# WZN1ng/Cooperative-Search

Hardware: AMD Instinct MI355X
Metric: env-steps/sec (higher is better)
Workload: dtype f64

## Files before the change

### cooperative-search_amd/csrc/rollout_oct.h

```cpp

#ifndef CS_OCT_PREFILTER
#define CS_OCT_PREFILTER 0
#endif
constexpr int OCT_WAVES = 3;
constexpr int OG = 8;
constexpr int OCT_ENVS = 64 / OG;
constexpr int OCT_BLOCK = 256;
constexpr int OCT_PAD = CS_MAX_AGENTS + 1;

struct __attribute__((aligned(16))) OctShared {
    double2 pos[OCT_ENVS][OCT_PAD];
    double2 tgt[OCT_ENVS][CS_MAX_TARGETS];
    float tile[OCT_ENVS * TILE_W];
    float reward[OCT_ENVS];
    int term[OCT_ENVS], win[OCT_ENVS];
    unsigned rowbuf[MT_N];
};

template <int LG>
struct OctLay;
template <>
struct OctLay<8> {
    static constexpr int ENVS = 8, TPL = 2;
    static constexpr unsigned SLICE = 0xffu;
// ... 96 lines not shown
};

struct OctKin {
    double cx, cy;
    double c1, s1;
    double xf, yf;
    bool hitf;
    bool hit;
};

__device__ __forceinline__ void div2_same_denominator(double nx, double ny, double den, double &qx, double &qy) {
    const double LO = 0x1p-100, HI = 0x1p100;
    const int e_lo = min(__builtin_amdgcn_frexp_exp(nx), __builtin_amdgcn_frexp_exp(ny));
    const bool plain = (den >= LO) & (den <= HI) & (fabs(nx) <= HI) & (fabs(ny) <= HI) & (e_lo >= -99);
    if (__builtin_expect(__ballot(!plain) == 0ull, 1)) {
        double r = __builtin_amdgcn_rcp(den);
        r = __builtin_fma(__builtin_fma(-den, r, 1.0), r, r);
        r = __builtin_fma(__builtin_fma(-den, r, 1.0), r, r);
        const double mx = nx * r, my = ny * r;
        qx = __builtin_fma(__builtin_fma(-den, mx, nx), r, mx);
        qy = __builtin_fma(__builtin_fma(-den, my, ny), r, my);
        return;
    }
    qx = nx / den;
    qy = ny / den;
}

template <int N, int I, bool SHARED_DIV, int LG = OG>
struct OctStage {
    static __device__ __forceinline__ void run(const DevParams &p, const double2 (&pre)[N], int t, bool act_lane,
                                               unsigned long long act_mask, OctKin &k) {
        if constexpr (I < N) {
            const double2 pi = pre[I];
            const double xi = pi.x, yi = pi.y;
            const double dx = k.cx - xi, dy = k.cy - yi;
            const double d2 = dx * dx + dy * dy;
            const bool c_lt = d2 < p.force_d2;
            const unsigned long long not_i = ~OctLay<LG>::lanes_t(I);
            if (__ballot(c_lt) & act_mask & not_i) {
                const bool c_nx = k.cx != xi, c_ny = k.cy != yi;
                const bool inr = act_lane & (t != I) & c_lt & (c_nx | c_ny);
                const double ex = -dx, ey = -dy;
                const double den = d2;
                double qx, qy;
                if constexpr (SHARED_DIV) {
                    div2_same_denominator(p.force_k * ex, p.force_k * ey, inr ? den : 1.0, qx, qy);
                } else {
                    qx = p.force_k * ex / den;
                    qy = p.force_k * ey / den;
                }
                const double tx = inr ? qx : 0.0;
                const double ty = inr ? qy : 0.0;
                double fx = 0.0, fy = 0.0;
                OctForceSum<N, I>::run(tx, ty, fx, fy);
                const double x = (k.cx + p.velocity * k.c1) + fx;
                const double y = (k.cy + p.velocity * k.s1) + fy;
                const bool h = (x < 0.0) | (x > p.L) | (y < 0.0) | (y > p.L);
                if (t == I) {
                    k.cx = h ? fmin(fmax(x, 0.0), p.L) : x;
                    k.cy = h ? fmin(fmax(y, 0.0), p.L) : y;
                    k.hit = h;
                }
            } else if (t == I) {
                k.cx = k.xf;
                k.cy = k.yf;
                k.hit = k.hitf;
            }
            OctStage<N, I + 1, SHARED_DIV, LG>::run(p, pre, t, act_lane, act_mask, k);
        }
    }
};

template <int N, bool SHARED_DIV = false, int LG = OG, int AP = OCT_PAD>
__device__ __forceinline__ unsigned oct_kinematics(const DevParams &p, const double *T, const double2 (*pos)[AP], int o, int t,
                                                   int sh8, bool stepping, int act, EnvO<N, LG> &e, int tl_step = -1) {
    static_assert(LG == OG, "one layout: the octet");
    const double PI = 3.141592653589793, TWO_PI = 2.0 * 3.141592653589793, THREE_PI = 3.0 * 3.141592653589793;
    const double DYAW = 3.141592653589793 / 18.0;
    const bool upd = (t < N) & stepping;
    double2 pre[N];
#pragma unroll
    for (int I = 0; I < N; I++) pre[I] = pos[o][I];
    double yaw = e.yaw;
    yaw = act == 1 ? yaw + DYAW : (act == 2 ? yaw + -DYAW : yaw);
    yaw = yaw > TWO_PI ? yaw - TWO_PI : (yaw < 0.0 ? yaw + TWO_PI : yaw);
    const double yw = yaw, yr = (yaw <= PI) ? PI - yaw : THREE_PI - yaw;
    double s1, c1, s2, c2;
    KIN_STAMP(3);
    if constexpr (N <= 4) {
        const double yr_up = dpp_f64<0x114>(yr);
        double sm, cm;
        trig_heading(T, t >= 4 ? yr_up : yw, sm, cm);
        s1 = sm;
        c1 = cm;
        s2 = dpp_f64<0x104>(sm);
        c2 = dpp_f64<0x104>(cm);
    } else {
        trig_heading_pair(T, yw, yr, s1, c1, s2, c2);
    }
    KIN_STAMP(4);
    const double xt = (e.x + p.velocity * c1) + 0.0, yt = (e.y + p.velocity * s1) + 0.0;
    const bool hitf = (xt < 0.0) | (xt > p.L) | (yt < 0.0) | (yt > p.L);
    OctKin k{e.x, e.y, c1, s1, hitf ? fmin(fmax(xt, 0.0), p.L) : xt, hitf ? fmin(fmax(yt, 0.0), p.L) : yt, hitf, false};
    constexpr bool FASTPATH = N <= 3;
    bool any_pair = !FASTPATH;
#pragma unroll
    for (int I = 0; I < (FASTPATH ? N : 0); I++) {
        const double2 pi = pre[I];
        const double qx = t < I ? k.xf : e.x, qy = t < I ? k.yf : e.y;
        const double dx = qx - pi.x, dy = qy - pi.y;
        any_pair = any_pair | ((t != I) & (dx * dx + dy * dy < p.force_d2) & ((qx != pi.x) | (qy != pi.y)));
    }
    const unsigned long long upd_mask = __ballot(upd);
    if (FASTPATH ? __ballot(any_pair & upd) != 0ull : upd_mask != 0ull) {
        OctStage<N, 0, SHARED_DIV, LG>::run(p, pre, t, upd, upd_mask, k);
    } else {
        k.cx = k.xf;
        k.cy = k.yf;
        k.hit = k.hitf;
    }
    KIN_STAMP(5);
    e.x = upd ? k.cx : e.x;
    e.y = upd ? k.cy : e.y;
    e.yaw = upd ? (k.hit ? yr : yw) : e.yaw;
    e.cs = upd ? (k.hit ? c2 : c1) : e.cs;
    e.sn = upd ? (k.hit ? s2 : s1) : e.sn;
    return oct_slice<LG>(__ballot(k.hit & upd), sh8);
}

__device__ __forceinline__ void tape_canon(unsigned (&t)[TAPE_DW], int &tcur) {
#pragma unroll
    for (int k = 0; k < TAPE_DW; k++) t[k] = __builtin_amdgcn_alignbit(k + 1 < TAPE_DW ? t[k + 1] : 0u, t[k], (unsigned)tcur);
    tcur = 0;
}
template <int N, int LG, int AP, bool LAZY, bool PRE = false>
__device__ __forceinline__ int oct_detect_impl(const DevParams &p, const double2 (*pos)[AP], int o, int t, int sh8, bool stepping,
                                               EnvO<N, LG> &e, unsigned (&tape)[TAPE_DW], int &tcur, const float *nrow = nullptr,
                                               int nstride = 0) {
    constexpr int MAXDW = (N * CS_MAX_TARGETS) / 32 < 1 ? 1 : (N * CS_MAX_TARGETS) / 32;
    constexpr int TPL = OctLay<LG>::TPL;
    static_assert(!PRE || TPL == 2, "the packed pre-filter holds a lane's two targets in one register pair");
    bool has[TPL], inr[N][TPL];
    unsigned below[TPL];
    int rank[N][TPL];
    int base = 0;
#pragma unroll
    for (int k = 0; k < TPL; k++) {
        has[k] = stepping & (t + LG * k < p.n_targets);
        below[k] = (1u << (t + LG * k)) - 1u;
    }
    auto exact = [&]() __attribute__((always_inline)) {
#pragma unroll
        for (int i = 0; i < N; i++) {
            const double2 a = pos[o][i];
#pragma unroll
            for (int k = 0; k < TPL; k++) {
                const double dx = e.tx[k] - a.x, dy = e.ty[k] - a.y;
                inr[i][k] = has[k] & (dx * dx + dy * dy <= p.view_r2);
            }
        }
    };
    if constexpr (PRE) {
        typedef float pk2 __attribute__((ext_vector_type(2)));
        const pk2 tnx = {e.tnx[0], e.tnx[1]}, tny = {e.tny[0], e.tny[1]};
        const float thr = p.thr32;
        float margin = 3.0e38f;
#pragma unroll
        for (int i = 0; i < N; i++) {
            const float ax = nrow[nstride * i], ay = nrow[nstride * i + 1];
            const pk2 dx = tnx - pk2{ax, ax}, dy = tny - pk2{ay, ay};
            const pk2 d2 = __builtin_elementwise_fma(dx, dx, dy * dy);
            const pk2 u = d2 - pk2{thr, thr};
            inr[i][0] = has[0] & (u[0] < 0.0f);
            inr[i][1] = has[1] & (u[1] < 0.0f);
            margin = __builtin_fminf(margin, __builtin_fminf(__builtin_fabsf(u[0]), __builtin_fabsf(u[1])));
        }
#ifndef CS_PREFILTER_EPS_SCALE
#define CS_PREFILTER_EPS_SCALE 1.0f
#endif
        if (__builtin_expect(__ballot(margin <= p.eps32 * CS_PREFILTER_EPS_SCALE) != 0ull, 0)) exact();
    } else {
        exact();
    }
#pragma unroll
    for (int i = 0; i < N; i++) {
        unsigned gm = 0u;
#pragma unroll
        for (int k = 0; k < TPL; k++) gm |= oct_slice<LG>(__ballot(inr[i][k]), sh8) << (LG * k);
#pragma unroll
        for (int k = 0; k < TPL; k++) rank[i][k] = base + __popc(gm & below[k]);
        base += __popc(gm);
    }
    unsigned w4[4];
#pragma unroll
    for (int k = 0; k < 4; k++) w4[k] = LAZY ? __builtin_amdgcn_alignbit(tape[k + 1], tape[k], (unsigned)tcur) : tape[k];
    const unsigned long long t64a = (unsigned long long)w4[0] | ((unsigned long long)w4[1] << 32);
    const unsigned long long t64b = (unsigned long long)w4[2] | ((unsigned long long)w4[3] << 32);
    auto slot = [&](int r) __attribute__((always_inline)) {
        if (N * CS_MAX_TARGETS <= 64) return (bool)((t64a >> r) & 1ull);
        return (bool)(((r >= 64 ? t64b : t64a) >> (r & 63)) & 1ull);
    };
    bool hit[TPL];
#pragma unroll
    for (int k = 0; k < TPL; k++) hit[k] = false;
    if (N * CS_MAX_TARGETS <= 64 || __builtin_expect(__ballot(base > 64) == 0ull, 1)) {
#pragma unroll
        for (int i = 0; i < N; i++)
#pragma unroll
            for (int k = 0; k < TPL; k++) hit[k] = hit[k] | (inr[i][k] & (bool)((t64a >> rank[i][k]) & 1ull));
    } else {
#pragma unroll
        for (int i = 0; i < N; i++)
#pragma unroll
            for (int k = 0; k < TPL; k++) hit[k] = hit[k] | (inr[i][k] & slot(rank[i][k]));
    }
    e.mt_pos = wrap624(e.mt_pos + 2 * base);
    e.words += (unsigned long long)(2 * base);
    e.ahead -= 2 * base;
    if constexpr (LAZY) {
        tcur += base;
#pragma unroll
        for (int r = 0; r <= MAXDW; r++) {
            const bool out = tcur >= 32;
            if (__ballot(out) == 0ull) break;
#pragma unroll
            for (int k = 0; k < TAPE_DW; k++) tape[k] = out ? (k + 1 < TAPE_DW ? tape[k + 1] : 0u) : tape[k];
            tcur -= out ? 32 : 0;
        }
    } else {
        tape_shift<MAXDW>(tape, base);
    }
    unsigned newly = 0u;
#pragma unroll
    for (int k = 0; k < TPL; k++) {
        const bool nw = hit[k] & !((e.found >> (t + LG * k)) & 1u);
        newly |= oct_slice<LG>(__ballot(nw), sh8) << (LG * k);
    }
    int r = 0;
    if (stepping) {
        const int cnt = __popc(newly);
        r = -1 + 10 * cnt;
        e.found |= newly;
        e.newly = newly;
        e.target_find += cnt;
        if (cnt > 0 && e.target_find == p.n_targets && !(e.flags & FLAG_WIN)) {
            r += 100;
            e.flags |= FLAG_WIN;
        }
        r -= __popc(((unsigned)e.flags >> 8) & 0xffu);
        e.curr_reward = r;
        e.flags |= FLAG_DIRTY;
    }
    return r;
}
template <int N, int LG = OG, int AP = OCT_PAD>
__device__ __forceinline__ int oct_detect(const DevParams &p, const double2 (*pos)[AP], int o, int t, int sh8, bool stepping,
                                          EnvO<N, LG> &e, unsigned (&tape)[TAPE_DW]) {
    int zero = 0;
    return oct_detect_impl<N, LG, AP, false>(p, pos, o, t, sh8, stepping, e, tape, zero);
}

template <int N, bool DRAIN = true, int LG = OG>
__device__ __forceinline__ void oct_wave_advance(const DevParams &p, int wave_b0, int nvalid, int lane, int min_ahead,
                                                 unsigned *rowbuf, EnvO<N, LG> &e, unsigned (&tape)[TAPE_DW], bool &tape_ok) {
    const int o = OctLay<LG>::valid(lane) ? OctLay<LG>::env(lane) : -1;
#pragma unroll 1
    for (int g = 0; g < OctLay<LG>::ENVS; g++) {
        const int pos = __shfl(e.mt_pos, OctLay<LG>::first_of(g)), a = __shfl(e.ahead, OctLay<LG>::first_of(g));
        const int ok = __shfl(tape_ok ? 1 : 0, OctLay<LG>::first_of(g));
        if (g >= nvalid || (ok && a >= min_ahead)) continue;
        unsigned *m = p.mt + (size_t)(wave_b0 + g) * MT_STRIDE;
        RowRegs rr;
        row_load(m, lane, rr);
        row_to_lds(rr, rowbuf, lane);
        row_twist_ahead(rowbuf, m, pos, a < 0 ? 0 : a, lane);
        unsigned long long bms[TAPE_DW / 2];
        row_hits_all(p, rowbuf, pos, lane, bms);
#pragma unroll
        for (int it = 0; it < TAPE_DW / 2; it++) {
            const unsigned long long bm = bms[it];
            if (o == g) {
                tape[2 * it] = (unsigned)(bm & 0xffffffffull);
                tape[2 * it + 1] = (unsigned)(bm >> 32);
            }
        }
        if (o == g) {
            e.ahead = MT_N;
            tape_ok = true;
        }
    }
    if (DRAIN) drain_vmem();
}


template <int N, int LG = OG>
__device__ __forceinline__ void oct_advance_finish(const DevParams &p, int wave_b0, int g, int lane, unsigned *rowbuf,
                                                   EnvO<N, LG> &e, unsigned (&tape)[TAPE_DW], bool &tape_ok) {
    const int o = OctLay<LG>::valid(lane) ? OctLay<LG>::env(lane) : -1;
    const int pos = __shfl(e.mt_pos, OctLay<LG>::first_of(g)), a = __shfl(e.ahead, OctLay<LG>::first_of(g));
    row_twist_ahead(rowbuf, p.mt + (size_t)(wave_b0 + g) * MT_STRIDE, pos, a < 0 ? 0 : a, lane);
    unsigned long long bms[TAPE_DW / 2];
    row_hits_all(p, rowbuf, pos, lane, bms);
#pragma unroll
    for (int it = 0; it < TAPE_DW / 2; it++) {
        const unsigned long long bm = bms[it];
        if (o == g) {
            tape[2 * it] = (unsigned)(bm & 0xffffffffull);
            tape[2 * it + 1] = (unsigned)(bm >> 32);
        }
    }
    if (o == g) {
        e.ahead = MT_N;
        tape_ok = true;
    }
}

template <int N, bool DRAIN, int LG = OG, class BeforeTile, class Pre>
__device__ __forceinline__ void oct_place_targets(const DevParams &cp, int wave_b0, int nvalid, int lane, bool live,
                                                  unsigned long long need, const double *rtab, double2 (*slots)[G], float *tile,
                                                  int W, unsigned *rowbuf, EnvO<N, LG> &e, unsigned (&tape)[TAPE_DW], bool &tape_ok,
                                                  BeforeTile before_tile, Pre pre) {
    using Lay = OctLay<LG>;
    const CS_AS4 DevParams *q = cold_params4();
    const int t16 = lane & (G - 1), gshift16 = lane & ~(G - 1), grp = lane >> 4, sh8 = Lay::first(lane), t = Lay::t(lane);
    const int n_targets = q->n_targets, target_mode = q->target_mode;
    const unsigned deter_mask = q->deter_mask;
    const double mid = q->mid, inv_half = q->inv_half, L = q->L;
    const CS_AS1 unsigned *mt = (const CS_AS1 unsigned *)q->mt;
    CS_AS1 double *tgt = (CS_AS1 double *)q->tgt;
    const unsigned tmask = n_targets >= 32 ? ~0u : ((1u << n_targets) - 1u);
    const unsigned fmask = target_mode == 0 ? ~deter_mask & tmask : 0u;
    const int need_total = __popc(fmask);
    const bool jit = (fmask >> t16) & 1u;
    const int my_rank = __popc(fmask & ((1u << t16) - 1u));
    unsigned long long pend = need;
    int taken_env = 0;
    bool first = true;
    while (pend) {
        const bool pending = Lay::valid(lane) && ((pend >> sh8) & 1ull);
        if (__ballot(live && pending && e.ahead < 4 * G))
            oct_wave_advance<N, DRAIN, LG>(cp, wave_b0, nvalid, lane, 4 * G, rowbuf, e, tape, tape_ok);
        unsigned long long m = pend;
        for (int k = 0; k < grp; k++) m &= m ? m - 1 : 0ull;
        const int src = m ? __ffsll((long long)m) - 1 : -1;
        const int sl = src >= 0 ? src : lane;
        const int g_pos = __shfl(e.mt_pos, sl), g_taken = __shfl(taken_env, sl);
        double px = 0.0, py = 0.0;
        if (__ballot(src >= 0 && g_taken > 0)) {
            const int from = src >= 0 ? src + (t16 % LG) : lane;
#pragma unroll
            for (int k = 0; k < Lay::TPL; k++) {
                const double xk = __shfl(e.tx[k], from), yk = __shfl(e.ty[k], from);
                if (t16 / LG == k) {
                    px = xk;
                    py = yk;
                }
            }
        }
        int words = 0, taken_new = 0;
        bool fin = false;
        if (src >= 0) {
            const int br = wave_b0 + Lay::env_of_first(src);
            double mx = rtab[t16], my = rtab[G + t16];
            fin = true;
            if (target_mode != 0 || need_total > 0) {
                unsigned w[4];
                if (!(first && pre(w))) {
                    const CS_AS1 unsigned *row = mt + (size_t)br * MT_STRIDE + wrap624(g_pos + 4 * t16);
#pragma unroll
                    for (int k = 0; k < 4; k++) w[k] = row[k];
                }
#pragma unroll
                for (int k = 0; k < 4; k++) w[k] = mt_temper(w[k]);
                const double u1 = ((double)(w[0] >> 5) * 67108864.0 + (double)(w[1] >> 6)) / 9007199254740992.0;
                const double u2 = ((double)(w[2] >> 5) * 67108864.0 + (double)(w[3] >> 6)) / 9007199254740992.0;
                if (target_mode == 0) {
                    if (g_taken > 0) {
                        mx = px;
                        my = py;
                    }
                    const double x1 = 2.0 * u1 - 1.0, x2 = 2.0 * u2 - 1.0;
                    const double r2 = x1 * x1 + x2 * x2;
                    const bool accept = !(r2 >= 1.0 || r2 == 0.0);
                    const double f = sqrt(-2.0 * log(accept ? r2 : 0.5) / (accept ? r2 : 0.5));
                    const double g1 = f * x2, g2 = f * x1;
                    const unsigned amask = (unsigned)((__ballot(accept) >> gshift16) & 0xffffull);
                    const int have = __popc(amask);
                    const int want = need_total - g_taken;
                    const int k = my_rank - g_taken;
                    const int sel = kth_set_bit16(amask, (k >= 0 && k < 16) ? k : 0);
                    const double s1 = __shfl(g1, sel & 15, G), s2 = __shfl(g2, sel & 15, G);
                    if (jit && k >= 0 && k < have && k < want) {
                        mx += rtab[2 * G + t16] * (s1 - 0.5);
                        my += rtab[3 * G + t16] * (s2 - 0.5);
                    }
                    const int last = have >= want ? kth_set_bit16(amask, want - 1) : 15;
                    words = 4 * (last + 1);
                    taken_new = g_taken + (have < want ? have : want);
                    fin = taken_new >= need_total;
                } else {
                    mx = L * u1;
                    my = L * u2;
                    words = 4 * n_targets;
                }
            }
            slots[grp][t16] = make_double2(mx, my);
            if (fin) {
                typedef double v2d __attribute__((ext_vector_type(2)));
                reinterpret_cast<CS_AS1 v2d *>(tgt + (size_t)br * G * 2)[t16] = v2d{mx, my};
                before_tile();
                if (t16 < n_targets) {
                    float *rs = tile + Lay::env_of_first(src) * W + 4 * N + 3 * t16;
                    rs[0] = (float)((mx - mid) * inv_half);
                    rs[1] = (float)((my - mid) * inv_half);
                    rs[2] = 0.0f;
                }
            }
        }
        __builtin_amdgcn_fence(__ATOMIC_RELEASE, "wavefront");
        __builtin_amdgcn_wave_barrier();
        __builtin_amdgcn_fence(__ATOMIC_ACQUIRE, "wavefront");
        const int rank = __popcll(pend & ((1ull << sh8) - 1ull));
        const bool got = pending && rank < 4;
        const int leader = got ? G * rank : lane;
        const int r_words = __shfl(words, leader), r_taken = __shfl(taken_new, leader), r_fin = __shfl(fin ? 1 : 0, leader);
        if (got) {
#pragma unroll
            for (int k = 0; k < Lay::TPL; k++) {
                const double2 tk = slots[rank][(t + LG * k) & (G - 1)];
                e.tx[k] = tk.x;
                e.ty[k] = tk.y;
            }
            oct_norm_targets<N, LG>(mid, inv_half, n_targets, t, e);
            tape_shift<1>(tape, r_words >> 1);
            e.mt_pos = wrap624(e.mt_pos + r_words);
            e.words += (unsigned long long)r_words;
            e.ahead -= r_words;
            taken_env = r_taken;
        }
        __builtin_amdgcn_fence(__ATOMIC_RELEASE, "wavefront");
        __builtin_amdgcn_wave_barrier();
        pend &= ~__ballot(got && r_fin != 0 && t == 0);
        first = false;
    }
}

template <int N, bool VEC, bool EMIT>
__global__ __launch_bounds__(OCT_BLOCK, OCT_WAVES) void k_rollout_oct(DevParams p, StepIO io) {
    __shared__ double T[TRIG_ROWS * TRIG_COLS];
    __shared__ OctShared shared[OCT_BLOCK / 64];
    __shared__ double rtab[4 * G];
    const int lane = threadIdx.x & 63, wave = __builtin_amdgcn_readfirstlane(threadIdx.x >> 6);
    const int o = lane >> 3, sh8 = lane & ~(OG - 1);
    int t = lane & (OG - 1);
    const int wave_b0 = io.env0 + (blockIdx.x * (OCT_BLOCK / 64) + wave) * OCT_ENVS;
    const int b_end = io.env0 + io.env_n;
    const int b = wave_b0 + o;
    const bool live = VEC || b < b_end;
    const int nvalid = b_end - wave_b0 < OCT_ENVS ? b_end - wave_b0 : OCT_ENVS;
    const int W = 4 * N + 3 * p.n_targets;
    bool ag = t < N;
    const bool auto_reset = io.flags & CS_AUTO_RESET, freeze = io.flags & CS_FREEZE_DONE;
    OctShared &sh = shared[wave];
    EnvO<N> e;
    const size_t bl = live ? (size_t)b : (size_t)io.env0;
    {
        const int4 *h4 = reinterpret_cast<const int4 *>(p.hdr + bl * CS_H_WORDS);
        const int4 h0 = h4[0], h1 = h4[1], h2 = h4[2];
        e.found = (unsigned)h0.x;
        e.newly = (unsigned)h0.y;
        e.target_find = h0.z;
        e.flags = h0.w;
        e.time_step = h1.x;
        e.total_reward = h1.y;
        e.mt_pos = h1.z;
        e.episodes = h1.w;
        e.words = (unsigned long long)(unsigned)h2.x | ((unsigned long long)(unsigned)h2.y << 32);
        e.curr_reward = h2.z;
        e.newly_reset = (unsigned)h2.w;
        e.ahead = p.ahead[bl];
        const double4 a = reinterpret_cast<const double4 *>(p.agent + bl * CS_MAX_AGENTS * 4)[t];
        e.x = a.x;
        e.y = a.y;
        e.yaw = a.z;
        const double2 *t2 = reinterpret_cast<const double2 *>(p.tgt + bl * G * 2);
        const double2 ta = t2[t], tb = t2[t + OG];
        e.tx[0] = ta.x;
        e.ty[0] = ta.y;
        e.tx[1] = tb.x;
        e.ty[1] = tb.y;
        oct_norm_targets<N, OG>(p, t, e);
    }
    const TapeRaw traw = tape_fetch(p, (int)bl);
    const int aidx = ag ? t : N - 1;
    const int astride = (io.flags & CS_ACTIONS_I64) ? 2 : 1;
    const int *ap = reinterpret_cast<const int *>(io.actions) + (bl * N + aidx) * astride;
    const size_t astep = (size_t)p.B * N * astride;
    int act = ap[0];
// ... 207 lines not shown
```

### cooperative-search_amd/csrc/rollout_od.h

```cpp

constexpr int OD_BLOCK = 128;
constexpr int OD_WAVES = 4;
constexpr int OD_SHARED_DIV_FROM_N = 99;
constexpr int ODE_SHARED_DIV_FROM_N = 5;
constexpr int od_ring(bool e3) { return e3 ? 8 : 4; }
static_assert((od_ring(false) & (od_ring(false) - 1)) == 0 && od_ring(false) >= 2, "ring depth");
static_assert((od_ring(true) & (od_ring(true) - 1)) == 0 && od_ring(true) >= 2, "ring depth");

template <int ENVS, int AP>
struct __attribute__((aligned(16))) OdRingT {
    double2 pos[ENVS][AP];
    double yaw[ENVS][AP - 1];
    float2 cssn[ENVS][AP - 1];
    unsigned out[ENVS];
    unsigned pad[ENVS];
};
template <int RING, int ENVS = OCT_ENVS, int AP = OCT_PAD, int TW = TILE_W>
struct __attribute__((aligned(16))) OdSharedT {
    OdRingT<ENVS, AP> ring[RING];
    double2 kpos[ENVS][AP];
    union {
        double2 dpos[ENVS][AP];
        float2 dnp[ENVS][AP];
    };
// ... 190 lines not shown
            __builtin_amdgcn_fence(__ATOMIC_ACQUIRE, "wavefront");
        };
        BLK_STAMP(1);
        const int *const abase = reinterpret_cast<const int *>(io.actions) + (bl * N + aidx) * astride;
        auto handle_fix = [&](int produced) __attribute__((always_inline)) {
            const int req = peek(&sh.fix_req);
            if (__builtin_expect(req != fix_seen, 0)) {
                __builtin_amdgcn_fence(__ATOMIC_ACQUIRE, "wavefront");
                const int fs = req - 1;
                const bool mine = live && ((sh.fix_mask >> o) & 1u);
                if (mine) {
                    const OdRing &r = sh.ring[fs & (OD_RING - 1)];
                    const double2 xy = r.pos[o][t];
                    e.x = xy.x;
                    e.y = xy.y;
                    e.yaw = r.yaw[o][t];
                    trig_heading(T, e.yaw, e.sn, e.cs);
                    sh.kpos[o][tc] = xy;
                    k_out = r.out[o];
                    k_done = true;
                }
                __builtin_amdgcn_fence(__ATOMIC_RELEASE, "wavefront");
                __builtin_amdgcn_wave_barrier();
                __builtin_amdgcn_fence(__ATOMIC_ACQUIRE, "wavefront");
                for (int j = fs + 1; j < produced; j++) produce(j, abase[(size_t)j * astep], mine, []() {});
                fix_seen = req;
                post(&sh.fix_ack, req);
            }
        };
        constexpr int OFF_FIX = (int)(offsetof(OdShared, fix_req) - offsetof(OdShared, d_steps)) / 4;
        constexpr int OFF_E = (int)(offsetof(OdShared, e_steps) - offsetof(OdShared, d_steps)) / 4;
        for (int s = 0; s < io.T; s++) {
            asm volatile("" : "+v"(t));
            ag = t < N;
            DUO_STAMP(0);
            OD_JITTER(1);
            const int act_after = ap[0];
            if (s + 3 < io.T) ap += astep;
            const int2 pv = E3 ? lds_peek2<OFF_E, OFF_FIX>(&sh.d_steps) : lds_peek2<0, OFF_FIX>(&sh.d_steps);
            if (__builtin_expect(pv.x <= s - OD_RING || pv.y != fix_seen, 0)) {
                for (;;) {
                    const int prog = peek(E3 ? &e_steps : &sh.d_steps);
                    handle_fix(s);
                    if (prog > s - OD_RING) break;
                    SPIN_TICK;
                    __builtin_amdgcn_s_sleep(2);
                }
            }
            DUO_STAMP(2);
            produce(s, act, true, []() {});
            DUO_STAMP(1);
            OD_JITTER(2);
            post(&sh.k_steps, s + 1);
            act = act_next;
            act_next = act_after;
        }
        BLK_STAMP(2);
        SPIN_STORE(0);
        while (peek(&sh.d_steps) < io.T - 1) {
            handle_fix(io.T);
            __builtin_amdgcn_s_sleep(4);
        }
        handle_fix(io.T);
        if (live && ag)
            reinterpret_cast<double4 *>(cold_params().agent + (size_t)b * CS_MAX_AGENTS * 4)[t] = make_double4(e.x, e.y, e.yaw, 0.0);
        BLK_STAMP(3);
        return;
    }

    if (E3 && role == 2) {
        const double2 *t2 = reinterpret_cast<const double2 *>(p.tgt + bl * G * 2);
        double2 tk[Lay::TPL];
#pragma unroll
        for (int k = 0; k < Lay::TPL; k++) tk[k] = t2[(t + LG * k) & (G - 1)];
        load_trig_to_lds(T);
        float *row = sh.tile + o * W;
#pragma unroll
        for (int k = 0; k < Lay::TPL; k++) {
            if (t + LG * k < p.n_targets) {
                row[4 * N + 3 * (t + LG * k) + 0] = (float)((tk[k].x - p.mid) * p.inv_half);
                row[4 * N + 3 * (t + LG * k) + 1] = (float)((tk[k].y - p.mid) * p.inv_half);
            }
        }
        auto peek = [](const int *w) __attribute__((always_inline)) { return lds_peek(w); };
        constexpr int W_MAX = 4 * N + 3 * CS_MAX_TARGETS;
        constexpr int Q = (ENVS * W_MAX / 4 + 63) / 64;
        const int ol = lane < ENVS * N ? lane : ENVS * N - 1;
        const int orow = ol / N, oag = ol - orow * N;
        const int obs_lds = orow * W + 4 * oag;
        const int rtw = lane < ENVS ? lane : ENVS - 1;
        float *p_rew = io.reward + wave_b0 + rtw;
        uint8_t *p_term = io.terminated + wave_b0 + rtw, *p_win = io.win + wave_b0 + rtw;
        v4f *p_obs = reinterpret_cast<v4f *>(io.obs + (size_t)wave_b0 * N * 4) + ol;
        v4f *p_st = reinterpret_cast<v4f *>(io.state + (size_t)wave_b0 * W);
        int chunk[Q];
#pragma unroll
        for (int q = 0; q < Q; q++) chunk[q] = lane + 64 * q < ENVS * W / 4 - 1 ? lane + 64 * q : ENVS * W / 4 - 1;
        int rf_served = 0;
        auto rf_serve = [&]() __attribute__((always_inline)) {
            const int seq = peek(&rf.rf_req);
            if (__builtin_expect(seq == rf_served, 1)) return;
            __builtin_amdgcn_fence(__ATOMIC_ACQUIRE, "wavefront");
            const int g = __builtin_amdgcn_readfirstlane(rf.rf_env), pos = __builtin_amdgcn_readfirstlane(rf.rf_pos);
            const int a = __builtin_amdgcn_readfirstlane(rf.rf_ahead);
            unsigned *m = cold_params().mt + (size_t)(wave_b0 + g) * MT_STRIDE;
            RowRegs rr;
            row_load(m, lane, rr);
            row_to_lds(rr, rf.erow, lane);
            row_twist_ahead(rf.erow, m, pos, a < 0 ? 0 : a, lane);
            unsigned long long bms[TAPE_DW / 2];
            row_hits_all(cold_params(), rf.erow, pos, lane, bms);
#pragma unroll
            for (int it = 0; it < TAPE_DW / 2; it++) {
                const unsigned long long bm = bms[it];
                if (lane == 0) {
                    rf.rf_tape[2 * it] = (unsigned)(bm & 0xffffffffull);
                    rf.rf_tape[2 * it + 1] = (unsigned)(bm >> 32);
                }
            }
            drain_vmem();
            {
                const int s = seq;
                (void)s;
                OD_JITTER(11);
            }
            __builtin_amdgcn_fence(__ATOMIC_RELEASE, "wavefront");
            if (lane == 0) lds_post(&rf.rf_done, seq);
            rf_served = seq;
        };
        for (int s = 0; s < io.T; s++) {
            asm volatile("" : "+v"(t));
            ag = t < N;
            OD_JITTER(3);
            if (EREF) rf_serve();
            while (peek(&sh.d_steps) <= s) {
                if (EREF) rf_serve();
                SPIN_TICK;
                __builtin_amdgcn_s_sleep(1);
            }
            OD_JITTER(4);
            __builtin_amdgcn_fence(__ATOMIC_ACQUIRE, "wavefront");
            const OdRing &r = sh.ring[s & (OD_RING - 1)];
            const OdOut &d = outs[s & (OD_RING - 1)];
            if (ag) {
                const double2 xy = r.pos[o][t];
                const float2 cs = r.cssn[o][t];
                row[4 * t + 0] = (float)((xy.x - p.mid) * p.inv_half);
                row[4 * t + 1] = (float)((xy.y - p.mid) * p.inv_half);
                row[4 * t + 2] = cs.x;
                row[4 * t + 3] = cs.y;
            }
            const unsigned found = d.found[o];
#pragma unroll
            for (int k = 0; k < Lay::TPL; k++)
                if (t + LG * k < p.n_targets) row[4 * N + 3 * (t + LG * k) + 2] = ((found >> (t + LG * k)) & 1u) ? 1.0f : 0.0f;
            const float o_rew = d.reward[rtw];
            const int o_term = d.term[rtw], o_win = d.win[rtw];
            __builtin_amdgcn_fence(__ATOMIC_RELEASE, "wavefront");
            __builtin_amdgcn_wave_barrier();
            __builtin_amdgcn_fence(__ATOMIC_ACQUIRE, "wavefront");
            v4f o_obs, o_st[Q];
            {
                const float *src = sh.tile + obs_lds;
                o_obs = v4f{src[0], src[1], src[2], src[3]};
                const float4 *src4 = reinterpret_cast<const float4 *>(sh.tile);
#pragma unroll
                for (int q = 0; q < Q; q++) {
                    const float4 v = src4[chunk[q]];
                    o_st[q] = v4f{v.x, v.y, v.z, v.w};
                }
            }
            __builtin_amdgcn_fence(__ATOMIC_ACQUIRE, "wavefront");
            *p_rew = o_rew;
            *p_term = (uint8_t)o_term;
            *p_win = (uint8_t)o_win;
            p_rew += p.B;
            p_term += p.B;
            p_win += p.B;
            __builtin_nontemporal_store(o_obs, p_obs);
            p_obs += (size_t)p.B * N;
#pragma unroll
            for (int q = 0; q < Q; q++) __builtin_nontemporal_store(o_st[q], p_st + chunk[q]);
            p_st += (size_t)p.B * W / 4;
            __builtin_amdgcn_fence(__ATOMIC_RELEASE, "wavefront");
            OD_JITTER(5);
            if (lane == 0) lds_post(&e_steps, s + 1);
        }
        if (EREF) {
            for (;;) {
                rf_serve();
                if (peek(&rf.d_done)) break;
                __builtin_amdgcn_s_sleep(2);
            }
        }
        SPIN_STORE(2);
        return;
    }

    if (!E3) __builtin_amdgcn_s_setprio(1);
    if (E3) __builtin_amdgcn_s_setprio(2);
    e.ahead = live ? p.ahead[bl] : (1 << 20);
    {
        const double2 *t2 = reinterpret_cast<const double2 *>(p.tgt + bl * G * 2);
#pragma unroll
        for (int k = 0; k < Lay::TPL; k++) {
            const double2 tk = t2[(t + LG * k) & (G - 1)];
            e.tx[k] = tk.x;
            e.ty[k] = tk.y;
        }
        oct_norm_targets<N, LG>(p, t, e);
    }
    const TapeRaw traw = tape_fetch(p, (int)bl);
    if (lane == 0) {
        sh.k_steps = 0;
        sh.d_steps = 0;
        sh.fix_req = 0;
        sh.fix_ack = 0;
        sh.fix_mask = 0u;
        e_steps = 0;
        rf.rf_req = 0;
        rf.rf_done = 0;
        rf.d_done = 0;
    }
    load_reset_tab(sh.rtab, lane);
    load_trig_to_lds(T);
    unsigned tape[TAPE_DW];
    bool tape_ok = tape_finish(p, traw, e, tape) || !live;
    int tcur = 0;
    auto canon = [&]() __attribute__((always_inline)) { tape_canon(tape, tcur); };
    float *row = sh.tile + o * W;
    auto put_found = [&]() __attribute__((always_inline)) {
#pragma unroll
        for (int k = 0; k < Lay::TPL; k++)
            if (t + LG * k < p.n_targets) row[4 * N + 3 * (t + LG * k) + 2] = ((e.found >> (t + LG * k)) & 1u) ? 1.0f : 0.0f;
    };
    if (!E3) {
#pragma unroll
        for (int k = 0; k < Lay::TPL; k++) {
            if (t + LG * k < p.n_targets) {
                row[4 * N + 3 * (t + LG * k) + 0] = (float)((e.tx[k] - p.mid) * p.inv_half);
                row[4 * N + 3 * (t + LG * k) + 1] = (float)((e.ty[k] - p.mid) * p.inv_half);
            }
        }
        put_found();
    }
    auto peek = [](const int *w) __attribute__((always_inline)) { return lds_peek(w); };
    auto post = [&](int *w, int v) __attribute__((always_inline)) {
        __builtin_amdgcn_fence(__ATOMIC_RELEASE, "wavefront");
        if (lane == 0) lds_post(w, v);
    };
    constexpr int LOW = 2 * N * CS_MAX_TARGETS;
#ifndef CS_OD_ASYNC
#define CS_OD_ASYNC 1
#endif
    constexpr int REQ_SLACK = 64;
    constexpr int REQ = CS_OD_ASYNC ? LOW + REQ_SLACK : 0;
    constexpr int W_MAX = 4 * N + 3 * CS_MAX_TARGETS;
    constexpr int Q = (ENVS * W_MAX / 4 + 63) / 64;
    constexpr int STEP_STORES = 3 + 1 + Q;
    static_assert(Q >= 1 && STEP_STORES == 4 + Q, "STEP_STORES counts the stores of the VEC && EMIT step: keep it next to them");
    auto wait_for_requests = [&]() __attribute__((always_inline)) {
#ifdef CS_OD_SAFE_WAIT
        drain_vmem();
#else
        if (!E3 && EMIT && VEC && STEP_STORES <= 15) __builtin_amdgcn_s_waitcnt(0x0F70 | STEP_STORES);
        else drain_vmem();
#endif
        __builtin_amdgcn_fence(__ATOMIC_ACQUIRE, "wavefront");
    };
    int k_seen = 0;
    int cand = -1;
    int ack_wait = 0;
    int rf_seq = 0, rf_pending = -1;
    unsigned long long rf_words0 = 0ull;
    auto rf_poll = [&](bool wait) __attribute__((always_inline)) {
        if (rf_pending < 0) return;
        if (wait) {
            {
                const int s = rf_seq;
                (void)s;
                OD_JITTER(12);
            }
            while (peek(&rf.rf_done) != rf_seq) __builtin_amdgcn_s_sleep(1);
        } else if (peek(&rf.rf_done) != rf_seq) {
            return;
        }
        __builtin_amdgcn_fence(__ATOMIC_ACQUIRE, "wavefront");
        canon();
        unsigned nt[TAPE_DW];
#pragma unroll
        for (int k = 0; k < TAPE_DW; k++) nt[k] = rf.rf_tape[k];
        const int c = (int)((e.words - rf_words0) >> 1);
        tape_shift<8>(nt, c);
        if (o == rf_pending) {
#pragma unroll
            for (int k = 0; k < TAPE_DW; k++) tape[k] = nt[k];
            e.ahead = MT_N - 2 * c;
            tape_ok = true;
        }
        rf_pending = -1;
    };
    unsigned long long pre_need = 0ull;
    unsigned pre_valid = 0u;
    oct_wave_advance<N, false, LG>(p, wave_b0, nvalid, lane, io.min_ahead > LOW ? io.min_ahead : LOW, sh.rowbuf, e, tape, tape_ok);
    const int rows_valid = nvalid;
    const int ol = lane < rows_valid * N ? lane : rows_valid * N - 1;
    const int orow = ol / N, oag = ol - orow * N;
    const int obs_lds = orow * W + 4 * oag;
    const int rtw = lane < rows_valid ? lane : rows_valid - 1;
    const int t16 = lane & (G - 1), gshift16 = lane & ~(G - 1), grp = lane >> 4;
    float *p_rew = io.reward + wave_b0 + rtw;
    uint8_t *p_term = io.terminated + wave_b0 + rtw, *p_win = io.win + wave_b0 + rtw;
    v4f *p_obs = reinterpret_cast<v4f *>(io.obs + (size_t)wave_b0 * N * 4) + ol;
    v4f *p_st = reinterpret_cast<v4f *>(io.state + (size_t)wave_b0 * W);
    int chunk[Q];
#pragma unroll
    for (int q = 0; q < Q; q++) chunk[q] = lane + 64 * q < ENVS * W / 4 - 1 ? lane + 64 * q : ENVS * W / 4 - 1;
    BLK_STAMP(5);
    for (int s = 0; s < io.T; s++) {
        asm volatile("" : "+v"(t));
        ag = t < N;
        DUO_STAMP(8);
        if (__builtin_expect(cand >= 0, 0)) {
            wait_for_requests();
            canon();
            oct_advance_finish<N, LG>(cold_params(), wave_b0, cand, lane, sh.rowbuf, e, tape, tape_ok);
            cand = -1;
        }
        if (EREF) rf_poll(false);
        if (__builtin_expect(__ballot(live && e.ahead < LOW) != 0ull, 0)) {
            if (EREF) rf_poll(true);
            canon();
            if (!EREF || __ballot(live && e.ahead < LOW) != 0ull)
                oct_wave_advance<N, false, LG>(cold_params(), wave_b0, nvalid, lane, LOW, sh.rowbuf, e, tape, tape_ok);
        }
        bool done = e.target_find >= p.n_targets || e.time_step >= p.time_limit;
        e.flags &= ~(FLAG_DIRTY | FLAG_RESET_PASS);
        const unsigned long long need = __ballot(live && done && auto_reset && t == 0);
        if (__builtin_expect(need != 0ull, 0)) {
            DUO_STAMP(13);
            if (EREF) rf_poll(true);
            canon();
            const DevParams &cp = cold_params();
            const bool mine = Lay::valid(lane) && ((need >> sh8) & 1ull);
            const StartTab<N> st = start_tab<N>();
            oct_place_targets<N, false, LG>(cp, wave_b0, nvalid, lane, live, need, sh.rtab, sh.tgt, sh.tile, W, sh.rowbuf, e, tape, tape_ok,
                                                   [&]() __attribute__((always_inline)) {
                                                       if (E3) {
                                                           while (lds_peek(&e_steps) < s) __builtin_amdgcn_s_sleep(1);
                                                           __builtin_amdgcn_fence(__ATOMIC_ACQUIRE, "wavefront");
                                                       }
                                                   },
                                                   [&](unsigned (&w)[4]) __attribute__((always_inline)) {
                                                       const bool ok = CS_OD_ASYNC && need == pre_need && ((pre_valid >> grp) & 1u);
                                                       if (ok) {
                                                           wait_for_requests();
#pragma unroll
                                                           for (int k = 0; k < 4; k++) w[k] = sh.prebuf[64 * k + lane];
                                                       }
                                                       return ok;
                                                   });
            if (mine) {
                e.episodes += 1;
                e.found = 0;
                e.newly = 0;
                e.target_find = 0;
                e.time_step = 0;
                e.total_reward = 0;
                e.flags = 0;
                double sx, sy;
                start_pick<N>(st, ag ? t : 0, sx, sy);
                sh.dpos[o][tc] = make_double2(sx, sy);
            }
            DUO_STAMP(14);
            if (__ballot(live && e.ahead < LOW)) oct_wave_advance<N, false, LG>(cp, wave_b0, nvalid, lane, LOW, sh.rowbuf, e, tape, tape_ok);
            __builtin_amdgcn_fence(__ATOMIC_RELEASE, "wavefront");
            __builtin_amdgcn_wave_barrier();
            __builtin_amdgcn_fence(__ATOMIC_ACQUIRE, "wavefront");
            DUO_STAMP(15);
            bool near = false;
#pragma unroll
            for (int i = 0; i < N; i++) {
                const double sx = st.x[i], sy = st.y[i];
#pragma unroll
                for (int k = 0; k < Lay::TPL; k++) {
                    const double axk = e.tx[k] - sx, ayk = e.ty[k] - sy;
                    near = near | ((t + LG * k < cp.n_targets) & (axk * axk + ayk * ayk <= cp.view_r2));
                }
            }
            if (__ballot(mine && near)) {
                oct_detect<N, LG, AP>(p, sh.dpos, o, t, sh8, mine, e, tape);
                if (!E3) put_found();
            } else if (mine) {
                e.newly = 0u;
                e.curr_reward = -1;
                e.flags |= FLAG_DIRTY;
            }
            done = done && !mine;
            if (__ballot(live && e.ahead < LOW)) oct_wave_advance<N, false, LG>(cp, wave_b0, nvalid, lane, LOW, sh.rowbuf, e, tape, tape_ok);
        }
        const bool stepping = live && !(done && freeze);
        DUO_STAMP(9);
        OD_JITTER(6);
        if (__builtin_expect(ack_wait != 0, 0)) {
            OD_JITTER(10);
            while (peek(&sh.fix_ack) != ack_wait) __builtin_amdgcn_s_sleep(1);
            ack_wait = 0;
        }
        if (k_seen <= s) {
            while ((k_seen = peek(&sh.k_steps)) <= s) { SPIN_TICK; __builtin_amdgcn_s_sleep(1); }
        }
        OD_JITTER(7);
        __builtin_amdgcn_fence(__ATOMIC_ACQUIRE, "wavefront");
        const OdRing &r = sh.ring[s & (OD_RING - 1)];
        if (live) e.flags = (e.flags & ~0xff00) | (int)(r.out[o] << 8);
#ifndef CS_OD_PREFILTER
#define CS_OD_PREFILTER 1
#endif
        constexpr bool PRE = CS_OD_PREFILTER == 2 || (CS_OD_PREFILTER == 1 && !E3);
        if ((!E3 || PRE) && ag) {
            const double2 xy = r.pos[o][t];
            const float nx = (float)((xy.x - p.mid) * p.inv_half), ny = (float)((xy.y - p.mid) * p.inv_half);
            if (!E3) {
                const float2 cs = r.cssn[o][t];
                row[4 * t + 0] = nx;
                row[4 * t + 1] = ny;
                row[4 * t + 2] = cs.x;
                row[4 * t + 3] = cs.y;
            } else {
                sh.dnp[o][t] = make_float2(nx, ny);
            }
        }
        if (PRE) {
            __builtin_amdgcn_fence(__ATOMIC_RELEASE, "wavefront");
            __builtin_amdgcn_wave_barrier();
            __builtin_amdgcn_fence(__ATOMIC_ACQUIRE, "wavefront");
        }
        const int reward = oct_detect_impl<N, LG, AP, true, PRE>(p, r.pos, o, t, sh8, stepping, e, tape, tcur,
                                                                                 E3 ? &sh.dnp[o][0].x : row, E3 ? 2 : 4);
        DUO_STAMP(10);
        bool term = true, mispredicted = false;
        if (stepping) {
            e.total_reward += reward;
            e.time_step += 1;
            term = e.target_find >= p.n_targets || e.time_step >= p.time_limit;
            mispredicted = (auto_reset || freeze) && term && e.time_step < p.time_limit;
        }
        const unsigned long long mb = s + 1 < io.T ? __ballot(mispredicted && t == 0) : 0ull;
        if (__builtin_expect(mb != 0ull, 0)) {
            unsigned m8 = 0;
#pragma unroll
            for (int q = 0; q < ENVS; q++) m8 |= (unsigned)((mb >> Lay::first_of(q)) & 1ull) << q;
            if (lane == 0) sh.fix_mask = m8;
            OD_JITTER(8);
            post(&sh.fix_req, s + 1);
        }
        if (E3) {
            if (t == 0) {
                OdOut &d = outs[s & (OD_RING - 1)];
                d.reward[o] = (float)reward;
                d.term[o] = term ? 1 : 0;
                d.win[o] = (e.flags & FLAG_WIN) ? 1 : 0;
                d.found[o] = e.found;
            }
        } else {
            if (__ballot(stepping && e.newly != 0u)) put_found();
            if (t == 0) {
                sh.reward[o] = (float)reward;
                sh.term[o] = term ? 1 : 0;
                sh.win[o] = (e.flags & FLAG_WIN) ? 1 : 0;
            }
            __builtin_amdgcn_fence(__ATOMIC_RELEASE, "wavefront");
            __builtin_amdgcn_wave_barrier();
            __builtin_amdgcn_fence(__ATOMIC_ACQUIRE, "wavefront");
        }
        float o_rew = 0.f;
        int o_term = 0, o_win = 0;
        if (!E3) {
            o_rew = sh.reward[rtw];
            o_term = sh.term[rtw];
            o_win = sh.win[rtw];
        }
        v4f o_obs = {0.f, 0.f, 0.f, 0.f}, o_st[Q];
        if (!E3 && (EMIT || io.obs)) {
            const float *src = sh.tile + obs_lds;
            o_obs = v4f{src[0], src[1], src[2], src[3]};
        }
        if (!E3 && VEC && (EMIT || io.state)) {
            const float4 *src4 = reinterpret_cast<const float4 *>(sh.tile);
#pragma unroll
            for (int q = 0; q < Q; q++) {
                const float4 v = src4[chunk[q]];
                o_st[q] = v4f{v.x, v.y, v.z, v.w};
            }
        }
        __builtin_amdgcn_fence(__ATOMIC_ACQUIRE, "wavefront");
        if (CS_OD_ASYNC && s + 1 < io.T) {
            const unsigned long long lowb = (EREF && rf_pending >= 0) ? 0ull : __ballot(live && e.ahead < REQ && t == 0);
            cand = lowb ? __builtin_amdgcn_readfirstlane(Lay::env_of_first(__ffsll((long long)lowb) - 1)) : -1;
            if (EREF && cand >= 0) {
                if (o == cand && t == 0) {
                    rf.rf_env = cand;
                    rf.rf_pos = e.mt_pos;
                    rf.rf_ahead = e.ahead;
                }
                rf_words0 = e.words;
                rf_pending = cand;
                rf_seq += 1;
                OD_JITTER(13);
                post(&rf.rf_req, rf_seq);
                cand = -1;
            }
            if (__builtin_expect(cand >= 0, 0)) {
                const unsigned *m = cold_params().mt + (size_t)(wave_b0 + cand) * MT_STRIDE;
#pragma unroll
                for (int i = 0; i < 10; i++)
                    __builtin_amdgcn_global_load_lds((const __attribute__((address_space(1))) void *)(m + lane + 64 * i),
                                                     (__attribute__((address_space(3))) void *)(sh.rowbuf + 64 * i), 4, 0, 0);
            }
            const unsigned long long nn = __ballot(live && stepping && term && auto_reset && t == 0);
            pre_need = nn;
            pre_valid = 0u;
            if (__builtin_expect(nn != 0ull, 0)) {
                unsigned long long mm = nn;
                for (int q = 0; q < grp; q++) mm &= mm ? mm - 1 : 0ull;
                const int src = mm ? __ffsll((long long)mm) - 1 : -1;
                const int sl = src >= 0 ? src : lane;
                const int ppos = __shfl(e.mt_pos, sl), pah = __shfl(e.ahead, sl);
                const bool okg = src >= 0 && pah >= 4 * G;
                if (okg) {
                    const unsigned *m = cold_params().mt + (size_t)(wave_b0 + Lay::env_of_first(src)) * MT_STRIDE;
                    const int i0 = wrap624(ppos + 4 * t16);
#pragma unroll
                    for (int q = 0; q < 4; q++)
                        __builtin_amdgcn_global_load_lds((const __attribute__((address_space(1))) void *)(m + wrap624(i0 + q)),
                                                         (__attribute__((address_space(3))) void *)(sh.prebuf + 64 * q), 4, 0, 0);
                }
                const unsigned long long vb = __ballot(okg);
                pre_valid = (unsigned)((vb >> 0) & 1ull) | ((unsigned)((vb >> 16) & 1ull) << 1) | ((unsigned)((vb >> 32) & 1ull) << 2) |
                            ((unsigned)((vb >> 48) & 1ull) << 3);
            }
        }
        if (!E3) {
            *p_rew = o_rew;
            *p_term = (uint8_t)o_term;
            *p_win = (uint8_t)o_win;
            p_rew += p.B;
            p_term += p.B;
            p_win += p.B;
        }
        if (!E3 && (EMIT || io.obs)) {
            __builtin_nontemporal_store(o_obs, p_obs);
            p_obs += (size_t)p.B * N;
        }
        if (!E3 && (EMIT || io.state)) {
            if (VEC) {
#pragma unroll
                for (int q = 0; q < Q; q++) __builtin_nontemporal_store(o_st[q], p_st + chunk[q]);
                p_st += (size_t)p.B * W / 4;
            } else {
                float *dst = io.state + ((size_t)s * p.B + wave_b0) * W;
                for (int k = lane; k < rows_valid * W; k += 64) dst[k] = sh.tile[k];
            }
        }
        DUO_STAMP(11);
        if (__builtin_expect(mb != 0ull, 0)) ack_wait = s + 1;
        OD_JITTER(9);
        post(&sh.d_steps, s + 1);
        DUO_STAMP(12);
    }
    BLK_STAMP(6);
    SPIN_STORE(1);
    if (EREF) {
        rf_poll(true);
        post(&rf.d_done, 1);
    }
    canon();
    if (live) {
        const DevParams &cp = cold_params();
        if (t == 0) {
// ... 18 lines not shown
```

Before: 538.5 million.

## Gate rare-path ballots on one summary mask and trim per-step found writes

```diff
diff --git a/cooperative-search_amd/csrc/rollout_oct.h b/cooperative-search_amd/csrc/rollout_oct.h
--- a/cooperative-search_amd/csrc/rollout_oct.h
+++ b/cooperative-search_amd/csrc/rollout_oct.h
@@ -202,7 +202,8 @@
 #pragma unroll
     for (int I = 0; I < N; I++) pre[I] = pos[o][I];
     double yaw = e.yaw;
-    yaw = act == 1 ? yaw + DYAW : (act == 2 ? yaw + -DYAW : yaw);
+    const double dyaw = act == 1 ? DYAW : (act == 2 ? -DYAW : -0.0);
+    yaw = yaw + dyaw;
     yaw = yaw > TWO_PI ? yaw - TWO_PI : (yaw < 0.0 ? yaw + TWO_PI : yaw);
     const double yw = yaw, yr = (yaw <= PI) ? PI - yaw : THREE_PI - yaw;
     double s1, c1, s2, c2;
@@ -323,7 +324,12 @@
     bool hit[TPL];
 #pragma unroll
     for (int k = 0; k < TPL; k++) hit[k] = false;
-    if (N * CS_MAX_TARGETS <= 64 || __builtin_expect(__ballot(base > 64) == 0ull, 1)) {
+    if (N <= 4 && (N * CS_MAX_TARGETS <= 32 || __builtin_expect(__ballot(base > 32) == 0ull, 1))) {
+#pragma unroll
+        for (int i = 0; i < N; i++)
+#pragma unroll
+            for (int k = 0; k < TPL; k++) hit[k] = hit[k] | (inr[i][k] & (bool)((w4[0] >> (rank[i][k] & 31)) & 1u));
+    } else if (N * CS_MAX_TARGETS <= 64 || __builtin_expect(__ballot(base > 64) == 0ull, 1)) {
 #pragma unroll
         for (int i = 0; i < N; i++)
 #pragma unroll
@@ -435,7 +441,7 @@
     }
 }
 
-template <int N, bool DRAIN, int LG = OG, class BeforeTile, class Pre>
+template <int N, bool DRAIN, int LG = OG, bool FLAGS = true, class BeforeTile, class Pre>
 __device__ __forceinline__ void oct_place_targets(const DevParams &cp, int wave_b0, int nvalid, int lane, bool live,
                                                   unsigned long long need, const double *rtab, double2 (*slots)[G], float *tile,
                                                   int W, unsigned *rowbuf, EnvO<N, LG> &e, unsigned (&tape)[TAPE_DW], bool &tape_ok,
@@ -533,7 +539,7 @@
                     float *rs = tile + Lay::env_of_first(src) * W + 4 * N + 3 * t16;
                     rs[0] = (float)((mx - mid) * inv_half);
                     rs[1] = (float)((my - mid) * inv_half);
-                    rs[2] = 0.0f;
+                    if (FLAGS) rs[2] = 0.0f;
                 }
             }
         }
diff --git a/cooperative-search_amd/csrc/rollout_od.h b/cooperative-search_amd/csrc/rollout_od.h
--- a/cooperative-search_amd/csrc/rollout_od.h
+++ b/cooperative-search_amd/csrc/rollout_od.h
@@ -296,6 +296,13 @@
                 row[4 * N + 3 * (t + LG * k) + 1] = (float)((tk[k].y - p.mid) * p.inv_half);
             }
         }
+        auto put_found = [&](unsigned found) __attribute__((always_inline)) {
+#pragma unroll
+            for (int k = 0; k < Lay::TPL; k++)
+                if (t + LG * k < p.n_targets) row[4 * N + 3 * (t + LG * k) + 2] = ((found >> (t + LG * k)) & 1u) ? 1.0f : 0.0f;
+        };
+        unsigned found_put = e.found;
+        put_found(found_put);
         auto peek = [](const int *w) __attribute__((always_inline)) { return lds_peek(w); };
         constexpr int W_MAX = 4 * N + 3 * CS_MAX_TARGETS;
         constexpr int Q = (ENVS * W_MAX / 4 + 63) / 64;
@@ -365,9 +372,10 @@
                 row[4 * t + 3] = cs.y;
             }
             const unsigned found = d.found[o];
-#pragma unroll
-            for (int k = 0; k < Lay::TPL; k++)
-                if (t + LG * k < p.n_targets) row[4 * N + 3 * (t + LG * k) + 2] = ((found >> (t + LG * k)) & 1u) ? 1.0f : 0.0f;
+            if (__builtin_expect(__ballot(found != found_put) != 0ull, 0)) {
+                put_found(found);
+                found_put = found;
+            }
             const float o_rew = d.reward[rtw];
             const int o_term = d.term[rtw], o_win = d.win[rtw];
             __builtin_amdgcn_fence(__ATOMIC_RELEASE, "wavefront");
@@ -458,7 +466,7 @@
         }
         put_found();
     }
-    auto peek = [](const int *w) __attribute__((always_inline)) { return lds_peek(w); };
+    auto peek = [](const int *w) __attribute__((always_inline)) { return __builtin_amdgcn_readfirstlane(lds_peek(w)); };
     auto post = [&](int *w, int v) __attribute__((always_inline)) {
         __builtin_amdgcn_fence(__ATOMIC_RELEASE, "wavefront");
         if (lane == 0) lds_post(w, v);
@@ -530,11 +538,14 @@
     int chunk[Q];
 #pragma unroll
     for (int q = 0; q < Q; q++) chunk[q] = lane + 64 * q < ENVS * W / 4 - 1 ? lane + 64 * q : ENVS * W / 4 - 1;
+    constexpr int RQ = REQ > LOW ? REQ : LOW;
+    unsigned long long rare = ~0ull;
     BLK_STAMP(5);
     for (int s = 0; s < io.T; s++) {
         asm volatile("" : "+v"(t));
         ag = t < N;
         DUO_STAMP(8);
+        const bool rare_top = rare != 0ull;
         if (__builtin_expect(cand >= 0, 0)) {
             wait_for_requests();
             canon();
@@ -542,7 +553,7 @@
             cand = -1;
         }
         if (EREF) rf_poll(false);
-        if (__builtin_expect(__ballot(live && e.ahead < LOW) != 0ull, 0)) {
+        if (__builtin_expect(rare_top && __ballot(live && e.ahead < LOW) != 0ull, 0)) {
             if (EREF) rf_poll(true);
             canon();
             if (!EREF || __ballot(live && e.ahead < LOW) != 0ull)
@@ -550,7 +561,7 @@
         }
         bool done = e.target_find >= p.n_targets || e.time_step >= p.time_limit;
         e.flags &= ~(FLAG_DIRTY | FLAG_RESET_PASS);
-        const unsigned long long need = __ballot(live && done && auto_reset && t == 0);
+        const unsigned long long need = rare_top ? __ballot(live && done && auto_reset && t == 0) : 0ull;
         if (__builtin_expect(need != 0ull, 0)) {
             DUO_STAMP(13);
             if (EREF) rf_poll(true);
@@ -558,10 +569,10 @@
             const DevParams &cp = cold_params();
             const bool mine = Lay::valid(lane) && ((need >> sh8) & 1ull);
             const StartTab<N> st = start_tab<N>();
-            oct_place_targets<N, false, LG>(cp, wave_b0, nvalid, lane, live, need, sh.rtab, sh.tgt, sh.tile, W, sh.rowbuf, e, tape, tape_ok,
+            oct_place_targets<N, false, LG, !E3>(cp, wave_b0, nvalid, lane, live, need, sh.rtab, sh.tgt, sh.tile, W, sh.rowbuf, e, tape, tape_ok,
                                                    [&]() __attribute__((always_inline)) {
                                                        if (E3) {
-                                                           while (lds_peek(&e_steps) < s) __builtin_amdgcn_s_sleep(1);
+                                                           while (peek(&e_steps) < s) __builtin_amdgcn_s_sleep(1);
                                                            __builtin_amdgcn_fence(__ATOMIC_ACQUIRE, "wavefront");
                                                        }
                                                    },
@@ -574,6 +585,7 @@
                                                        }
                                                        return ok;
                                                    });
+            pre_valid = 0u;
             if (mine) {
                 e.episodes += 1;
                 e.found = 0;
@@ -660,7 +672,8 @@
             term = e.target_find >= p.n_targets || e.time_step >= p.time_limit;
             mispredicted = (auto_reset || freeze) && term && e.time_step < p.time_limit;
         }
-        const unsigned long long mb = s + 1 < io.T ? __ballot(mispredicted && t == 0) : 0ull;
+        rare = __ballot(live & ((e.ahead < RQ) | (term & (auto_reset | (freeze & stepping)))));
+        const unsigned long long mb = (s + 1 < io.T && rare != 0ull) ? __ballot(mispredicted && t == 0) : 0ull;
         if (__builtin_expect(mb != 0ull, 0)) {
             unsigned m8 = 0;
 #pragma unroll
@@ -709,7 +722,7 @@
             }
         }
         __builtin_amdgcn_fence(__ATOMIC_ACQUIRE, "wavefront");
-        if (CS_OD_ASYNC && s + 1 < io.T) {
+        if (CS_OD_ASYNC && s + 1 < io.T && __builtin_expect(rare != 0ull, 0)) {
             const unsigned long long lowb = (EREF && rf_pending >= 0) ? 0ull : __ballot(live && e.ahead < REQ && t == 0);
             cand = lowb ? __builtin_amdgcn_readfirstlane(Lay::env_of_first(__ffsll((long long)lowb) - 1)) : -1;
             if (EREF && cand >= 0) {
```

Result: slower. 494.8 million (-8.1%).
